# LuisaGroup/LuisaRender

Hardware: AMD Instinct MI355X
Metric: Msamples/s (+ fraction of HBM roofline) at fixed SPP, 1/2/4/8 GPU (higher is better)
Workload: dtype f32; 1 GPU; Contemporary Bathroom-class (procedural stand-in, ~600k tris), 1024x1024, 1024spp, depth 16; integrator=MegaPath, sampler=Independent (seed 19980810), spp=1024, parallelism=single GPU, collective=none (single GPU), scheduler=path pool, two contexts per lane (megapool_kernel.h)

## Files before the change

__graft_entry__.py:

```python
import os
import subprocess
import sys

ROOT = os.path.dirname(os.path.abspath(__file__))
if ROOT not in sys.path:
    sys.path.insert(0, ROOT)


def build() -> None:
    jobs = f"-j{min(os.cpu_count() or 4, 16)}"
    subprocess.check_call(["make", "-C", ROOT, jobs, "host", "oracle", "hip", "cli", "ieee", "shallow", "noearly", "nopair", "noride", "nostraight"])
    if os.path.isdir("/root/reference/src"):
        subprocess.check_call(["make", "-C", ROOT, jobs, "ref"])
    import luisarender_amd
    from luisarender_amd import _ffi
    _ffi.host_lib()
    assert os.path.exists(os.path.join(ROOT, "luisarender_amd", "lib", "liblrhip.so"))


def smoke() -> None:
    import numpy as np
    from luisarender_amd import Scene
    from oracle.check import Oracle
    from luisarender_amd.render import MegaPathRenderer
    from luisarender_amd.scenes import cornell_box

    scene = Scene.from_string(cornell_box(resolution=64, spp=8))
    renderer = MegaPathRenderer(0)
    renderer.upload(scene)
    renderer.render(0, 8, counters=True, sync=True)
    gpu = renderer.download(converted=False)
    cpu, counters = Oracle(scene).render(0, 8)
    rel = float(np.abs(gpu[..., :3] - cpu[..., :3]).sum() / np.abs(cpu[..., :3]).sum())
    gc = renderer.counters()
    assert np.array_equal(gpu[..., 3], cpu[..., 3]), "sample counts differ"
    assert abs(gc["closest_rays"] - counters["closest_rays"]) <= 2, (gc, counters)
    assert rel < 1e-4, f"relative L1 vs oracle {rel}"
    print(f"smoke ok: rel L1 vs oracle = {rel:.3e}, {renderer.last_render_ms():.3f} ms")


if __name__ == "__main__":
    build()
    if len(sys.argv) > 1 and sys.argv[1] == "smoke":
        smoke()
```

luisarender_amd/csrc/hip/lrhip_render.hip:

```cpp
#include "lrhip_internal.h"

namespace lrh {

#ifndef LR_TAPER_BIG
#define LR_TAPER_BIG 2.5
#endif
#ifndef LR_TAPER_SMALL
#define LR_TAPER_SMALL 3.0
#endif
#ifndef LR_TAPER_FRACTION
#define LR_TAPER_FRACTION 0.9
#endif
Chunking chunking_of(uint32_t spp, double shard_tiles, double item_scale, bool taper) {
    const auto s_opt = std::max(1.0, std::sqrt(item_scale * spp * shard_tiles / kNominalWaves));
    Chunking c{};
    if (taper && spp >= 16u) {
        const auto big_min = static_cast<long>((static_cast<uint64_t>(spp) * 2u + kMaxChunks - 1u) / kMaxChunks);
        c.big = static_cast<uint32_t>(std::clamp(std::max(std::lround(LR_TAPER_BIG * s_opt), big_min), 1l, static_cast<long>(spp)));
        c.small = static_cast<uint32_t>(std::clamp(std::lround(s_opt / LR_TAPER_SMALL), 1l, static_cast<long>(c.big)));
        c.big_count = static_cast<uint32_t>(std::floor(LR_TAPER_FRACTION * spp / c.big));
        const auto rest = spp - c.big_count * c.big;
        auto small_count = (rest + c.small - 1u) / c.small;
        if (c.big_count + small_count > kMaxChunks && c.big_count < kMaxChunks) {
            c.small = (rest + (kMaxChunks - c.big_count) - 1u) / (kMaxChunks - c.big_count);
            small_count = (rest + c.small - 1u) / c.small;
        }
        c.count = c.big_count + small_count;
        if (c.big_count >= 1u && small_count >= 1u && c.count <= kMaxChunks) { return c; }
    }
    auto count = static_cast<uint32_t>(std::lround(spp / s_opt));
    count = std::max(1u, std::min({count, spp, kMaxChunks}));
    c.count = c.big_count = count, c.big = (spp + count - 1u) / count, c.small = c.big;
    return c;
}

constexpr int kMinFixedBits = 24;
int fixed_point_bits(float film_clamp, float shutter_weight, uint32_t spp) {
    const auto bound = std::max(1.0, static_cast<double>(film_clamp) * std::max(1.0,
        std::fabs(static_cast<double>(shutter_weight)))) * std::max(1u, spp);
    if (!std::isfinite(bound)) { return -1; }
    const auto bits = std::min(40, 61 - static_cast<int>(std::ceil(std::log2(bound))));
    return bits >= kMinFixedBits ? bits : -1;
}
int ensure_accum(lrhip_ctx *ctx, uint32_t pixel_count) {
    const auto bytes = static_cast<size_t>(pixel_count) * 3u * sizeof(unsigned long long);
    if (ctx->wf_accum.bytes < bytes) {
        if (auto r = ensure(ctx->wf_accum, bytes); r != LRHIP_OK) { return r; }
        LR_HIP_CHECK(hipMemsetAsync(ctx->wf_accum.ptr, 0, bytes, ctx->stream));
    }
    return LRHIP_OK;
}
constexpr uint32_t kPoolAutoTriangles = 98304u;
uint32_t pool_auto_triangles(uint32_t max_depth, uint32_t scene_spp) {
    auto t = kPoolAutoTriangles;
    if (max_depth <= 6u) { t *= 2u; }
    if (scene_spp != 0u && scene_spp < 64u) { t /= 2u; }
    return t;
}
bool wants_pool(const lrhip_ctx *ctx) {
    return ctx->scheduler == 2u || (ctx->scheduler == 0u && ctx->update_counts[1] >= pool_auto_triangles(ctx->scene.max_depth,
        ctx->scene.sampler_spp));
}
int ensure_pool(lrhip_ctx *ctx, uint32_t resident_blocks) {
    return ensure(ctx->pool, static_cast<size_t>(resident_blocks) * lrd::kWavesPerBlock * lrd::kPoolSlots * lrd::kPoolRecordQuadsMax
        * sizeof(float4));
}

}

using namespace lrh;

extern "C" {

int lrhip_render(lrhip_ctx *ctx, const lrhip_render_params *p) {
    if (ctx == nullptr || p == nullptr || !ctx->scene_ready) { return fail(LRHIP_ERROR_INVALID, "lrhip_render: no scene uploaded"); }
    auto tiles_x = (ctx->width + 7u) / 8u, tiles_y = (ctx->height + 7u) / 8u;
    auto tile_count = tiles_x * tiles_y;
    if (p->spp_end < p->spp_begin || p->tile_stride == 0u || p->tile_end > tile_count) {
        return fail(LRHIP_ERROR_INVALID, "lrhip_render: invalid spp/tile range");
    }
    LR_HIP_CHECK(hipSetDevice(ctx->device));
    ctx->timed = false;
    if (p->spp_end == p->spp_begin || p->tile_begin >= p->tile_end) { return LRHIP_OK; }
    if (!ctx->scene.has_lights && ctx->scene.env_kind == lrd::kEnvNone && ctx->scene.integrator_kind != LR_INTEGRATOR_NORMAL) {
        return LRHIP_OK;
    }
    auto tiles_in_range = (p->tile_end - p->tile_begin + p->tile_stride - 1u) / p->tile_stride;
    auto spp = p->spp_end - p->spp_begin;
    const auto weight = (p->flags & LRHIP_RENDER_SHUTTER_WEIGHT) != 0u ? p->shutter_weight : 1.f;
    const auto fixed_bits = fixed_point_bits(ctx->scene.film_clamp, weight, spp);
    PlanInputs in{};
    in.features = ctx->features, in.force_features = ctx->diag_force_features, in.sampler_kind = ctx->scene.sampler_kind;
    in.wf_mode = ctx->wf_mode, in.max_depth = ctx->scene.max_depth;
    in.count = (p->flags & LRHIP_RENDER_COUNTERS) != 0u, in.env_tree = ctx->env_tree, in.byte_texels = ctx->packed_texel_words != 0u;
    in.wants_pool = wants_pool(ctx), in.fixed_fits = fixed_bits >= 0;
    if (fixed_bits < 0 && !ctx->in_split && fixed_point_bits(ctx->scene.film_clamp, weight, 1u) >= 0) {
        auto fitting = in;
        fitting.fixed_fits = true;
        if (plan_kernels(fitting).fixed_point) {
            auto n = spp;
            while (n > 1u && fixed_point_bits(ctx->scene.film_clamp, weight, n) < 0) { n = (n + 1u) / 2u; }
            LR_HIP_CHECK(hipEventRecord(ctx->ev_begin, ctx->stream));
            struct SplitGuard {
                lrhip_ctx *c;
                ~SplitGuard() { c->in_split = false; }
            } guard{ctx};
            ctx->in_split = true;
            auto rc = LRHIP_OK;
            for (auto s0 = p->spp_begin; s0 < p->spp_end && rc == LRHIP_OK; s0 += n) {
                auto sub = *p;
                sub.spp_begin = s0, sub.spp_end = std::min(p->spp_end, s0 + n);
                rc = lrhip_render(ctx, &sub);
            }
            return rc;
        }
    }
    const auto plan = plan_kernels(in);
    if (plan.family == LRHIP_FAMILY_WAVEFRONT) { return render_wavefront(ctx, p, plan, tiles_x, tiles_y, tiles_in_range, tile_count); }
    auto shard_tiles = static_cast<double>(tile_count) / std::max(p->balance_shards, 1u);
    auto item_scale = 1.25;
    if (ctx->diag_item_scale != 0.) { item_scale *= std::max(0.01, std::fabs(ctx->diag_item_scale)); }
    const auto ck = chunking_of(spp, shard_tiles, item_scale, ctx->diag_item_scale >= 0.);
    const auto chunk_count = ck.count;
    lrd::RenderArgs args{};
    args.film = ctx->film;
    ctx->scene.shutter_weight = weight;
    args.spp_begin = p->spp_begin, args.spp_end = p->spp_end;
    args.tile_begin = p->tile_begin, args.tile_end = p->tile_end, args.tile_stride = p->tile_stride;
    args.tiles_x = tiles_x, args.tiles_y = tiles_y;
    args.chunk_count = chunk_count;
    args.chunk_big_count = ck.big_count, args.chunk_big = ck.big, args.chunk_small = ck.small;
    args.item_count = tiles_in_range * chunk_count;
    args.work_counter = static_cast<uint32_t *>(ctx->work_counter.ptr);
    args.spill = static_cast<uint32_t *>(ctx->spill.ptr);
    args.counters = static_cast<lrd::DCounters *>(ctx->counters.ptr);
    auto pixel_count = ctx->width * ctx->height;
    LR_HIP_CHECK(hipMemsetAsync(ctx->work_counter.ptr, 0, 1024u, ctx->stream));
    const auto aov = plan.family == LRHIP_FAMILY_AOV, pool = plan.family == LRHIP_FAMILY_POOL;
    const auto entry = plan.family != LRHIP_FAMILY_NONE ? find_kernel(plan.main) : nullptr;
    if (entry == nullptr) {
        if (aov) {
            return fail(LRHIP_ERROR_UNSUPPORTED, "lrhip_render: no AOV kernel for feature mask " + std::to_string(plan.main)
                + " was compiled into this library");
        }
        return fail(LRHIP_ERROR_UNSUPPORTED, "lrhip_render: no megakernel variant for feature mask " + std::to_string(ctx->features) +
                                                 " was compiled into this library");
    }
    const auto aov_channels = aov ? ctx->scene.aov_channels : 0u;
// ... 58 lines not shown
```

luisarender_amd/csrc/hip/megapool_kernel.h:

```cpp
#pragma once
#include "dev_wavefront.h"

namespace lrd {

#ifndef LR_MIN_WAVES
#define LR_MIN_WAVES 4
#endif
#ifndef LR_POOL_SHADE_LANES
#define LR_POOL_SHADE_LANES 56
#endif
#ifndef LR_POOL_IDLE_LANES
#define LR_POOL_IDLE_LANES 16
#endif
#ifndef LR_POOL_TURNOVER_LANES
#define LR_POOL_TURNOVER_LANES 12
#endif
#ifndef LR_POOL_PARK_ON_STACK
#define LR_POOL_PARK_ON_STACK 1
#endif
#ifndef LR_POOL_FUSED_FETCH
#define LR_POOL_FUSED_FETCH 1
#endif
#ifndef LR_POOL_FUSED_ALPHA
#define LR_POOL_FUSED_ALPHA 0
#endif
#ifndef LR_POOL_EARLY_FETCH
#define LR_POOL_EARLY_FETCH 1
#endif
#ifndef LR_POOL_LEAF_NODE_PAIR
#define LR_POOL_LEAF_NODE_PAIR 1
#endif
#ifndef LR_POOL_EARLY_TAIL_PRIO
#define LR_POOL_EARLY_TAIL_PRIO 3
#endif
#ifndef LR_POOL_STATE_LEAN
#define LR_POOL_STATE_LEAN 1
#endif
#ifndef LR_POOL_RAY_INIT
#define LR_POOL_RAY_INIT if (!mine)
#endif
#ifndef LR_POOL_SHADOW_RIDE
#define LR_POOL_SHADOW_RIDE 1
#endif
constexpr uint32_t kPoolSlots = 128u;

template<bool GENERIC>
constexpr uint32_t pool_quads() { return GENERIC ? 5u : 4u; }
constexpr uint32_t kPoolRecordQuadsMax = pool_quads<true>() + 1u;
constexpr uint32_t kPoolPending = 1u << 22u;

enum : uint32_t {
    kCtxShadow = 1u, kCtxClosest = 2u,
    kCtxHadShadow = 4u, kCtxHadClosest = 8u,
    kCtxDone = 16u,
    kCtxOccluded = 32u,
    kCtxSide = 64u,
    kCtxOpen = 128u,
};
struct PathCtx {
    f3 so, sd;
    float s_tmax;
    f3 no, nd;
    float n_tmin, n_tmax;
    uint32_t tri;
    float u, v;
    uint32_t flags;
};
LR_D void ctx_start(PathCtx &c, TravState &tr) {
    tr.o = c.no, tr.d = c.nd, tr.t_min = c.n_tmin, tr.t_max = c.n_tmax;
    tr.phase = kPhaseClosest;
    if ((c.flags & kCtxShadow) != 0u) {
        asm volatile("");
        tr.o = c.so, tr.d = c.sd, tr.t_min = 0.f, tr.t_max = c.s_tmax;
        tr.phase = kPhaseShadow;
        c.flags &= ~kCtxShadow;
    } else {
        asm volatile("");
        c.flags &= ~kCtxClosest;
    }
    tr.cur = 0u, tr.sp = 0u;
    tr.hit.tri = kInvalid, tr.hit.u = 0.f, tr.hit.v = 0.f;
    tr.occluded = false;
}

LR_D void swap_words(float &x, float &y) { asm volatile("v_swap_b32 %0, %1" : "+v"(x), "+v"(y)); }
LR_D void swap_words(uint32_t &x, uint32_t &y) { asm volatile("v_swap_b32 %0, %1" : "+v"(x), "+v"(y)); }
LR_D void ctx_swap(PathCtx &a, PathCtx &b) {
    swap_words(a.so.x, b.so.x), swap_words(a.so.y, b.so.y), swap_words(a.so.z, b.so.z), swap_words(a.s_tmax, b.s_tmax);
    swap_words(a.sd.x, b.sd.x), swap_words(a.sd.y, b.sd.y), swap_words(a.sd.z, b.sd.z);
    swap_words(a.no.x, b.no.x), swap_words(a.no.y, b.no.y), swap_words(a.no.z, b.no.z), swap_words(a.n_tmin, b.n_tmin);
    swap_words(a.nd.x, b.nd.x), swap_words(a.nd.y, b.nd.y), swap_words(a.nd.z, b.nd.z), swap_words(a.n_tmax, b.n_tmax);
    swap_words(a.tri, b.tri), swap_words(a.u, b.u), swap_words(a.v, b.v), swap_words(a.flags, b.flags);
}

#ifndef LR_POOL_TURNOVER_MOVES
#define LR_POOL_TURNOVER_MOVES 1
#endif
LR_D void ctx_turnover(PathCtx &a, PathCtx &b) {
    if (LR_POOL_TURNOVER_MOVES == 0) { ctx_swap(a, b); return; }
    a.so = b.so, a.sd = b.sd, a.s_tmax = b.s_tmax, a.n_tmin = b.n_tmin, a.n_tmax = b.n_tmax;
    b.tri = a.tri, b.u = a.u, b.v = a.v;
    swap_words(a.no.x, b.no.x), swap_words(a.no.y, b.no.y), swap_words(a.no.z, b.no.z);
    swap_words(a.nd.x, b.nd.x), swap_words(a.nd.y, b.nd.y), swap_words(a.nd.z, b.nd.z);
    swap_words(a.flags, b.flags);
}

LR_D uint32_t lane_rank(unsigned long long mask) {
    return __builtin_amdgcn_mbcnt_hi(static_cast<uint32_t>(mask >> 32u), __builtin_amdgcn_mbcnt_lo(static_cast<uint32_t>(mask), 0u));
}

constexpr uint32_t kCtxRays = kCtxShadow | kCtxClosest;
LR_D bool ctx_shadeable(uint32_t flags, bool samples_left) {
#ifdef LR_POOL_SINGLE
    if ((flags & kCtxSide) != 0u) { samples_left = false; }
#endif
    return (flags & kCtxDone) != 0u || (samples_left && (flags & kCtxOpen) == 0u);
}
LR_D bool pool_shade_due(uint32_t phase, uint32_t cur_flags, uint32_t oth_flags, bool samples_left) {
    const auto idle = phase == kPhaseIdle;
    const auto s = lr_ballot(ctx_shadeable(oth_flags, samples_left) || (idle && ctx_shadeable(cur_flags, samples_left)));
    if (s == 0ull) { return false; }
    const auto idle_mask = lr_ballot(idle);
    return static_cast<uint32_t>(__popcll(s)) >= static_cast<uint32_t>(LR_POOL_SHADE_LANES) ||
           static_cast<uint32_t>(__popcll(s & idle_mask)) >= static_cast<uint32_t>(LR_POOL_IDLE_LANES) || idle_mask == ~0ull;
}

template<bool COUNT, bool ALPHA>
// ... 57 lines not shown
            stats.steps_starved += static_cast<uint32_t>(__builtin_readcyclecounter() - probe_t2);
        }
#endif
        if (n_ended == 0u) { continue; }
        if (n_ended < static_cast<uint32_t>(LR_POOL_TURNOVER_LANES) && lr_any(tr.cur < kCurParked)) { continue; }
        if (ended) {
            if (tr.phase == kPhaseShadow) {
                if (tr.occluded) { cur.flags |= kCtxOccluded; }
            } else {
                cur.tri = tr.hit.tri, cur.u = tr.hit.u, cur.v = tr.hit.v;
            }
            tr.phase = kPhaseIdle, tr.cur = kCurIdle;
            if ((cur.flags & kCtxRays) == 0u) {
                cur.flags |= kCtxDone;
                if ((oth.flags & kCtxRays) != 0u) { ctx_turnover(cur, oth); }
            }
            if ((cur.flags & kCtxRays) != 0u) {
                ctx_start(cur, tr);
                inv = safe_inverse(tr.d);
                spb = tl.lds_base;
            }
        }
        if (!lr_any(ended && tr.cur == kCurIdle)) { continue; }
        if (lr_ballot(tr.cur != kCurIdle) == 0ull) { break; }
        if (pool_shade_due(tr.phase, cur.flags, oth.flags, samples_left)) { break; }
    }
    if (EARLY != 0) { trav_fetch_wait(); }
    LR_MARK(kProbeTail, tr.cur);
    prio_shade();
    tr.sp = tl.sp_of(spb);
    return for_alpha;
}

#ifndef LR_PADDED_DRAWS_OUT_OF_LINE
#define LR_PADDED_DRAWS_OUT_OF_LINE 1
#endif
struct PaddedDraws {
    float a, b, c, d;
};
[[maybe_unused]] static __device__ __noinline__ PaddedDraws padded_draws(const DScene *scene, uint32_t sample_index, uint32_t pixel, uint32_t dimension, bool four) {
    PathSampler<true> sampler{};
    uint32_t words[kWfSamplerWordsMax] = {sample_index, 0u, dimension, pixel};
    sampler.restore(*scene, words);
    PaddedDraws r;
    r.a = sampler.next_1d();
    const auto u = sampler.next_2d();
    r.b = u.x, r.c = u.y;
    r.d = four ? sampler.next_1d() : 0.f;
    return r;
}

#ifndef LR_LIGHT_OUT_OF_LINE
#if defined(LR_VARIANT) && ((LR_VARIANT) & 16) && !((LR_VARIANT) & (96 | 256))
#define LR_LIGHT_OUT_OF_LINE 1
#else
#define LR_LIGHT_OUT_OF_LINE 0
#endif
#endif
template<bool ENV>
[[maybe_unused]] static __device__ __noinline__ LightPick sample_one_light_call(const DScene *scene, f3 p, f3 ng, f3 ns, uint32_t offset_bits, float u0, float u1, float u2) {
    SurfacePoint it{};
    it.p = p, it.ng = ng, it.shading.n = ns, it.offset_bits = offset_bits;
    return sample_one_light<ENV>(*scene, it, u0, f2{u1, u2});
}

#define LR_POOL_FILM_ADD(L, PIXEL, OF_ITEM, TILE_PIXEL)                                                                                          \
    do {                                                                                                                                         \
        const auto rgb = (L) * scene.shutter_weight;                                                                                             \
        if (CONT || (OF_ITEM) != item) {                                \
            wf_film_accumulate(scene, args.film, (PIXEL), rgb, scene.film_clamp);                                                                \
        } else if (!(any_nan(rgb) || any_inf(rgb))) {   \
            const auto threshold = scene.film_clamp * fmaxf(1.f, 1.f);                                                                           \
            const auto strength = fmaxf(fmaxf(fmaxf(fabsf(rgb.x), fabsf(rgb.y)), fabsf(rgb.z)), 0.f);                                            \
            const auto c = rgb * (threshold / fmaxf(strength, threshold));                                                                       \
            const auto px_sums = film_tile + (TILE_PIXEL) * 3u;                                                                                  \
            if (c.x != 0.f) { atomicAdd(px_sums + 0, radiance_to_fixed(c.x, scene.wf.accum_scale)); }                                            \
            if (c.y != 0.f) { atomicAdd(px_sums + 1, radiance_to_fixed(c.y, scene.wf.accum_scale)); }                                            \
            if (c.z != 0.f) { atomicAdd(px_sums + 2, radiance_to_fixed(c.z, scene.wf.accum_scale)); }                                            \
        } else {                                                                        \
            atomicAdd(&args.film[(PIXEL)].w, -1.f);                                                                                              \
        }                                                                                                                                        \
    } while (false)

template<uint32_t F>
__global__ __launch_bounds__(kBlockThreads, LR_MIN_WAVES) void megapool_kernel(DScenePtr scene_ptr, RenderArgs args) {
    const DScene &scene = *(const DScene *)scene_ptr;
    constexpr bool COUNT = (F & kFeatCount) != 0u, PCG = (F & kFeatGeneric) != 0u, ENV = (F & kFeatEnv) != 0u,
                   ALPHA = (F & kFeatAlpha) != 0u, DISNEY = (F & kFeatDisney) != 0u, WF = (F & kFeatWf) != 0u, CONT = (F & kFeatCont) != 0u;
    static_assert((F & kFeatPool) != 0u, "a pool variant");
    static_assert(kPoolParkedWords == 5u, "the shading block parks five words on top of a lane's stack (below): lrhip_upload_scene bounds the BVH depth with this constant");
    static_assert((F & (kFeatMix | kFeatLayered | kFeatAux | kFeatVpt | kFeatNest)) == 0u, "the pool scheduler exists for the lean kernels (closures inline)");
    static_assert(!WF || !DISNEY, "a wavefront variant is a lean kernel: the heavy closures live in heavy_kernel.h");
    static_assert(!CONT || WF, "the continuation pass exists in wavefront mode only");
    constexpr uint32_t SAMPLER_WORDS = PathSampler<PCG>::kSavedWords;
#ifdef LR_ONLY_SAMPLER
    constexpr bool PADDED = PCG && (LR_ONLY_SAMPLER) == LR_SAMPLER_PADDED_SOBOL;
#else
    constexpr bool PADDED = false;
#endif
    static_assert(PADDED == ((F & kFeatPadded) != 0u) || (F & kFeatPadded) == 0u, "a kFeatPadded kernel: generic sampler, LR_ONLY_SAMPLER = PaddedSobol");
    constexpr uint32_t QUADS = PADDED ? 4u : pool_quads<PCG>();
    constexpr bool RIDE = LR_POOL_SHADOW_RIDE != 0 && !WF;
    constexpr uint32_t RECORD = QUADS + (RIDE ? 1u : 0u);
    static_assert(RECORD <= kPoolRecordQuadsMax, "ensure_pool sizes the records");
    __shared__ uint32_t s_stack[kStackLds * kBlockThreads];
    __shared__ float4 s_stage[kWavesPerBlock * kStageWave];
#if LR_POOL_PARK_ON_STACK == 0
    __shared__ uint32_t s_park[5u * kBlockThreads];
    static_assert(kStackLds + 5u <= 16u, "the parking area is carved out of the round 1-3 stack: compile such pool variants with LR_STACK_LDS <= 11");
#endif
    __shared__ unsigned long long s_film[CONT ? 1u : kWavesPerBlock * 192u];
#ifdef LR_STALL_PROBE
    __shared__ uint32_t s_probe[kWavesPerBlock * kProbeWords];
    if ((threadIdx.x & 63u) < kProbeWords) { s_probe[(threadIdx.x >> 6u) * kProbeWords + (threadIdx.x & 63u)] = 0u; }
    const auto probe_wave = (F & kFeatCount) != 0u && (blockIdx.x % 9u) == 0u && __builtin_amdgcn_readfirstlane(threadIdx.x >> 6u) == ((blockIdx.x / 9u) & 3u);
#endif
    const auto tid = threadIdx.x;
    const auto lane = tid & 63u;
    const auto gtid = blockIdx.x * kBlockThreads + tid;
    const auto wave_in_block = __builtin_amdgcn_readfirstlane(tid >> 6u);
    TraversalStack stack{s_stack + tid, args.spill + gtid, args.total_threads, s_stage + wave_in_block * kStageWave};
    const auto film_tile = s_film + (CONT ? 0u : wave_in_block * 192u);
    const auto state_of = [&](uint32_t side, uint32_t quad) { return args.pool + static_cast<size_t>(side * RECORD + quad) * args.total_threads + gtid; };
    const auto state_load = [&](uint32_t side, uint32_t quad) { return *state_of(side, quad); };
    const auto state_store = [&](uint32_t side, uint32_t quad, float4 v) { *state_of(side, quad) = v; };
    DCounters local{};
    const auto t_wave = COUNT ? __builtin_readcyclecounter() : 0ull;

    const auto cont_total = CONT ? min(scene.wf.counts[kWfCountCont], scene.wf.capacity) : 0u;
    const auto cont_waves = gridDim.x * kWavesPerBlock;
    const auto item_records = CONT ? min(kWfItemRecords, max(64u, ((cont_total + cont_waves - 1u) / cont_waves + 63u) & ~63u)) : 1u;
    const auto item_count = CONT ? (cont_total + item_records - 1u) / item_records : args.item_count;
    const auto cont_queue = wf_cont_queue(scene);

    auto item = kInvalid;
    auto items_left = true;
    auto q_next = 0u, q_total = 0u;
    auto s_begin = 0u, s_count = 0u, tx = 0u, ty = 0u;
    if (!CONT) { film_tile[lane * 3u] = 0ull, film_tile[lane * 3u + 1u] = 0ull, film_tile[lane * 3u + 2u] = 0ull; }
    TravState tr{};
    tr.phase = kPhaseIdle;
    PathCtx cur{}, oth{};
    cur.flags = 0u, oth.flags = kCtxSide;

    auto flush_tile = [&]() {
        if (CONT || item == kInvalid) { return; }
        __builtin_amdgcn_fence(__ATOMIC_ACQ_REL, "wavefront");
        __builtin_amdgcn_wave_barrier();
        const auto a0 = film_tile[lane * 3u], a1 = film_tile[lane * 3u + 1u], a2 = film_tile[lane * 3u + 2u];
        film_tile[lane * 3u] = 0ull, film_tile[lane * 3u + 1u] = 0ull, film_tile[lane * 3u + 2u] = 0ull;
        const auto wx = tx * 8u + (lane & 7u), wy = ty * 8u + (lane >> 3u);
        if (wx < scene.camera.width && wy < scene.camera.height) {
            const auto index = wy * scene.camera.width + wx;
            const auto acc = scene.wf.accum + static_cast<size_t>(index) * 3u;
            if (a0 != 0ull) { atomicAdd(acc + 0, a0); }
            if (a1 != 0ull) { atomicAdd(acc + 1, a1); }
            if (a2 != 0ull) { atomicAdd(acc + 2, a2); }
            if (s_count != 0u) { atomicAdd(&args.film[index].w, static_cast<float>(s_count)); }
        }
        __builtin_amdgcn_fence(__ATOMIC_ACQ_REL, "wavefront");
        __builtin_amdgcn_wave_barrier();
    };

    auto take_item = [&]() {
        flush_tile();
        item = next_item(CONT ? scene.wf.counts + kWfWorkCont : args.work_counter, item_count, lane);
        q_next = 0u, q_total = 0u, s_count = 0u;
        if (item == kInvalid) {
            items_left = false;
            return;
        }
        if (CONT) {
            q_total = min(item_records, cont_total - item * item_records);
        } else {
            const auto range = item_range(args, item);
            const auto tile = args.tile_begin + range.tile_index * args.tile_stride;
            ty = tile / args.tiles_x, tx = (tile - ty * args.tiles_x + ty) % args.tiles_x;
            s_begin = range.s_begin, s_count = range.s_end > range.s_begin ? range.s_end - range.s_begin : 0u;
            q_total = s_count * 64u;
        }
    };

    for (;;) {
        for (;;) {
            const auto samples_left = items_left || q_next < q_total;
            if (!pool_shade_due(tr.phase, cur.flags, oth.flags, samples_left)) { break; }
            const auto t_shade = COUNT ? __builtin_readcyclecounter() : 0ull;
            if (ALPHA) { tr.pend_t = 0.f, tr.pend_u = 0.f, tr.pend_v = 0.f; }
            if (tr.phase == kPhaseIdle && !ctx_shadeable(oth.flags, samples_left)) { ctx_swap(cur, oth); }
#ifdef LR_POOL_SINGLE
            const auto mine = (oth.flags & kCtxDone) != 0u || ((oth.flags & kCtxOpen) == 0u && (oth.flags & kCtxSide) == 0u);
#else
            const auto mine = (oth.flags & kCtxDone) != 0u || (oth.flags & kCtxOpen) == 0u;
#endif
            {
                const auto stage = stack.stage;
                stage[lane] = make_float4(cur.so.x, cur.so.y, cur.so.z, cur.s_tmax);
                stage[64u + lane] = make_float4(cur.sd.x, cur.sd.y, cur.sd.z, cur.n_tmin);
                stage[128u + lane] = make_float4(cur.no.x, cur.no.y, cur.no.z, cur.n_tmax);
                const auto keep_word = (tr.phase & 7u) | (tr.occluded ? 8u : 0u) | (tr.sp << 5u) | (cur.flags << 12u) | (oth.flags << 20u);
                stage[192u + lane] = make_float4(cur.nd.x, cur.nd.y, cur.nd.z, __uint_as_float(keep_word));
#if LR_POOL_PARK_ON_STACK
                stack.push(tr.sp + 0u, tr.phase != kPhaseIdle ? tr.hit.tri : cur.tri);
                stack.push(tr.sp + 1u, __float_as_uint(tr.phase != kPhaseIdle ? tr.hit.u : cur.u));
                stack.push(tr.sp + 2u, __float_as_uint(tr.phase != kPhaseIdle ? tr.hit.v : cur.v));
                stack.push(tr.sp + 3u, __float_as_uint(tr.t_max));
                stack.push(tr.sp + 4u, tr.cur);
#else
                const auto park = s_park + tid;
                park[0u * kBlockThreads] = tr.phase != kPhaseIdle ? tr.hit.tri : cur.tri;
                park[1u * kBlockThreads] = __float_as_uint(tr.phase != kPhaseIdle ? tr.hit.u : cur.u);
                park[2u * kBlockThreads] = __float_as_uint(tr.phase != kPhaseIdle ? tr.hit.v : cur.v);
                park[3u * kBlockThreads] = __float_as_uint(tr.t_max);
                park[4u * kBlockThreads] = tr.cur;
#endif
                asm volatile("" ::: "memory");
            }
            PathSampler<PCG> sampler{};
            Ray ray{}, shadow{};
            LR_POOL_RAY_INIT {
                shadow.o = oth.so, shadow.d = oth.sd, shadow.t_min = 0.f, shadow.t_max = oth.s_tmax;
                ray.o = oth.no, ray.d = oth.nd, ray.t_min = oth.n_tmin, ray.t_max = oth.n_tmax;
            }
            f3 beta = mk3(0.f), Li = mk3(0.f), nee = mk3(0.f);
            auto pdf_bsdf = 1e16f;
            auto dp = 0u, pixel_index = 0u, path_item = kInvalid;
            const auto side = (oth.flags & kCtxSide) != 0u ? 1u : 0u;
            auto path_open = (oth.flags & kCtxDone) != 0u;
            const auto traced_shadow = path_open && (oth.flags & kCtxHadShadow) != 0u, traced_closest = path_open && (oth.flags & kCtxHadClosest) != 0u;
            const auto occluded = (oth.flags & kCtxOccluded) != 0u;
            const auto ro = oth.no, rd = oth.nd;
            const auto hit_tri = oth.tri;
            const auto hit_u = oth.u, hit_v = oth.v;
            constexpr bool LEAN_STATE = LR_POOL_STATE_LEAN != 0;
            auto word0 = 0u;
            const auto load_ids = [&]() {
                const auto q3 = state_load(side, 3u);
                pixel_index = __float_as_uint(q3.x), path_item = __float_as_uint(q3.y);
            };
            const auto sampler_take = [&](uint32_t stage) {
                if (PADDED) {
                    const auto q3 = state_load(side, 3u);
                    const auto depth = dp & 0xffffu;
                    const auto first_rr = scene.rr_depth == 0u ? 0u : scene.rr_depth - 1u;
                    const auto dimension = (scene.camera.kind == LR_CAMERA_THIN_LENS ? 4u : 2u) + 6u * depth + (depth > first_rr ? depth - first_rr : 0u) + 3u * stage;
                    uint32_t words[kWfSamplerWordsMax] = {__float_as_uint(q3.z), 0u, dimension, __float_as_uint(q3.w)};
                    sampler.restore(scene, words);
                    return;
                }
                const auto q3 = state_load(side, 3u);
                uint32_t words[kWfSamplerWordsMax] = {word0, __float_as_uint(q3.z), __float_as_uint(q3.w), __float_as_uint(state_load(side, QUADS - 1u).x)};
                sampler.restore(scene, words);
            };
            const auto sampler_leave = [&]() {
                if (PADDED) { return; }
                uint32_t words[kWfSamplerWordsMax] = {0u, 0u, 0u, 0u};
                sampler.save(words);
                word0 = words[0];
                state_store(side, 2u, make_float4(Li.x, Li.y, Li.z, __uint_as_float(words[0])));
                const auto q3 = state_load(side, 3u);
                state_store(side, 3u, make_float4(q3.x, q3.y, __uint_as_float(words[1]), __uint_as_float(words[2])));
                state_store(side, QUADS - 1u, make_float4(__uint_as_float(words[3]), 0.f, 0.f, 0.f));
            };
            auto sampler_left = false;
            if (path_open) {
                const auto q0 = state_load(side, 0u), q1 = state_load(side, 1u), q2 = state_load(side, 2u);
                nee = mk3(q0.x, q0.y, q0.z), pdf_bsdf = q0.w;
                beta = mk3(q1.x, q1.y, q1.z);
                const auto packed = __float_as_uint(q1.w);
                dp = packed & (RIDE ? 0x7fffffu : 0x3fffffu);
                Li = mk3(q2.x, q2.y, q2.z);
                word0 = __float_as_uint(q2.w);
                if (!LEAN_STATE) { load_ids(); }
                if (!PCG) {
                    uint32_t words[kWfSamplerWordsMax] = {word0, 0u, 0u, 0u};
                    sampler.restore(scene, words);
                }
            }
            auto want_shadow = false, want_closest = false;
            unsigned long long t_closure_sum = 0ull;
#ifdef LR_STALL_PROBE
            uint32_t t_lobe = 0u, t_eval = 0u, t_sample = 0u, t_hit = 0u, t_light = 0u;
            const auto probe_clock = []() { return static_cast<uint32_t>(__builtin_readcyclecounter()); };
            const auto t_block = probe_clock();
#endif
            auto park_kind = kInvalid;
            if (path_open) {
                if (traced_shadow) {
                    if (!occluded) { Li += nee; }
                }
                if (RIDE && (dp & kPoolPending) != 0u) {
                    const auto ids = state_load(side, QUADS);
                    LR_POOL_FILM_ADD(Li, __float_as_uint(ids.x), __float_as_uint(ids.y), __float_as_uint(ids.z));
                    Li = mk3(0.f), nee = mk3(0.f);
                    dp &= ~kPoolPending;
                }
                if (traced_closest) {
                    if (COUNT) { local.shade_busy++; }
                    const auto wo = -rd;
// ... 95 lines not shown
#endif
                        const LobeTables tables{scene.closures, scene.surfaces, scene.textures, scene.texels};
                        DClosure closure;
                        Frame sh;
                        load_lobe(tables, it.uv, it.ng, wo, (it.tags >> 12u) & 4095u, it.shading, closure, sh);
#ifdef LR_STALL_PROBE
                        asm volatile("" : "+v"(closure.c0[0]), "+v"(closure.s0), "+v"(sh.n.x));
                        const auto t_l1 = probe_clock();
                        t_lobe = t_l1 - static_cast<uint32_t>(t_closure);
#endif
                        if (pick.pdf > 0.0f) {
                            const auto eval = closure_evaluate<DISNEY>(closure, sh, it.ng, wo, shadow.d);
                            const auto w = balance(pick.pdf, eval.pdf) / pick.pdf;
                            nee = w * beta * eval.f * pick.L;
                            want_shadow = nee.x != 0.f || nee.y != 0.f || nee.z != 0.f;
                        }
#ifdef LR_STALL_PROBE
                        asm volatile("" : "+v"(nee.x), "+v"(nee.y), "+v"(nee.z));
                        const auto t_e1 = probe_clock();
                        t_eval = t_e1 - t_l1;
#endif
                        if constexpr (PADDED && LR_PADDED_DRAWS_OUT_OF_LINE != 0) {
                            sampler_take(1u);
                            const auto r = padded_draws(&scene, sampler.lo, sampler.w3, sampler.w2, rr);
                            u_lobe = r.a, u_bsdf = f2{r.b, r.c}, u_rr = r.d;
                        } else {
                            if (PCG) { sampler_take(1u); }
                            u_lobe = sampler.next_1d();
                            u_bsdf = sampler.next_2d();
                            if (PCG) {
                                if (rr) { u_rr = sampler.next_1d(); }
                                sampler_leave();
                            }
                        }
                        const auto bs = closure_sample<DISNEY>(closure, sh, it.ng, wo, u_lobe, u_bsdf);
                        auto eta = 1.f;
                        const auto has_eta = closure_eta(closure, eta);
                        ray.o = robust_origin(it, bs.wi);
                        ray.d = bs.wi;
                        ray.t_min = 0.f, ray.t_max = kFloatMax;
                        pdf_bsdf = bs.pdf;
                        beta *= (bs.pdf > 0.f ? 1.f / bs.pdf : 0.f) * bs.f;
                        auto eta_scale = 1.f;
                        if (has_eta) {
                            if (bs.event == kEventEnter) { eta_scale = sqr(eta); }
                            else if (bs.event == kEventExit) { eta_scale = sqr(1.f / eta); }
                        }
                        if (any_nan(beta)) { beta = mk3(0.f); }
                        auto alive = !(beta.x <= 0.f && beta.y <= 0.f && beta.z <= 0.f);
                        if (!PCG && rr) { u_rr = sampler.next_1d(); }
                        if (alive) {
                            const auto q = fmaxf(max_component(beta) * eta_scale, .05f);
                            if (rr) {
                                if (q < scene.rr_threshold && u_rr >= q) { alive = false; }
                                else { beta *= q < scene.rr_threshold ? 1.0f / q : 1.f; }
                            }
                        }
                        dp++;
                        want_closest = alive && (dp & 0xffffu) < scene.max_depth;
                        if (COUNT) { t_closure_sum += __builtin_readcyclecounter() - t_closure; }
#ifdef LR_STALL_PROBE
                        asm volatile("" : "+v"(beta.x), "+v"(ray.d.x));
                        t_sample = probe_clock() - t_e1;
#endif
                    }
                }
            }
            if (WF) {
                if (park_kind != kInvalid) { path_open = false; }
            }
            if (path_open && !want_shadow && !want_closest) {
                if (LEAN_STATE) { load_ids(); }
                LR_POOL_FILM_ADD(Li, pixel_index, path_item, dp >> 16u);
                path_open = false;
            }
            const auto t_regen = COUNT ? __builtin_readcyclecounter() : 0ull;
            if (COUNT) {
                for (auto off = 32; off > 0; off >>= 1) { t_closure_sum = max(t_closure_sum, static_cast<unsigned long long>(__shfl_xor(static_cast<long long>(t_closure_sum), off))); }
            }
            const auto final_shadow = RIDE && path_open && want_shadow && !want_closest;
            auto need = mine && (!path_open || final_shadow);
            auto got = false;
            auto new_k = 0u, new_item = kInvalid, new_px = 0u, new_py = 0u, new_s = 0u;
            for (;;) {
                const auto mask = lr_ballot(need);
                if (mask == 0ull) { break; }
                if (q_next >= q_total) {
                    if (!items_left) { break; }
                    take_item();
                    if (!items_left) { break; }
                    continue;
                }
                const auto avail = q_total - q_next;
                const auto rank = lane_rank(mask);
                if (need && rank < avail) {
                    const auto k = q_next + rank;
                    const auto px = tx * 8u + (k & 7u), py = ty * 8u + ((k >> 3u) & 7u);
                    if (CONT || (px < scene.camera.width && py < scene.camera.height)) {
                        new_k = k, new_item = item, new_px = px, new_py = py, new_s = s_begin + (k >> 6u);
                        got = true, need = false;
                    }
                }
                q_next += min(static_cast<uint32_t>(__popcll(mask)), avail);
            }
            if (got) {
                sampler_left = false;
                if (CONT) {
                    const auto rec = new_item * item_records + new_k;
                    const auto &q = cont_queue;
                    ray.o = q.get3(rec, 0u), ray.d = q.get3(rec, 3u);
                    ray.t_min = 0.f, ray.t_max = kFloatMax;
                    shadow.o = q.get3(rec, 6u), shadow.d = q.get3(rec, 9u);
                    shadow.t_min = 0.f, shadow.t_max = q.getf(rec, 12u);
                    nee = q.get3(rec, 13u), beta = q.get3(rec, 16u), Li = q.get3(rec, 19u);
                    pdf_bsdf = q.getf(rec, 22u);
                    pixel_index = q.get(rec, 23u);
                    const auto packed = q.get(rec, 24u);
                    dp = packed & 0xffffu;
                    want_shadow = (packed & (1u << 16u)) != 0u, want_closest = (packed & (1u << 17u)) != 0u;
                    uint32_t words[kWfSamplerWordsMax];
#pragma unroll
                    for (auto w = 0u; w < SAMPLER_WORDS; w++) { words[w] = q.get(rec, kWfContWords + w); }
                    sampler.restore(scene, words);
                    path_open = true;
                } else {
                    if (final_shadow) {
                        if (LEAN_STATE) { load_ids(); }
                        state_store(side, QUADS, make_float4(__uint_as_float(pixel_index), __uint_as_float(path_item), __uint_as_float(dp >> 16u), 0.f));
                    }
                    pixel_index = new_py * scene.camera.width + new_px;
                    path_item = new_item;
                    sampler.start(scene, new_px, new_py, new_s);
                    const auto u_filter = sampler.next_pixel_2d();
                    const auto u_lens = scene.camera.kind == LR_CAMERA_THIN_LENS ? sampler.next_2d() : f2{.5f, .5f};
                    float weight;
                    camera_ray(scene, scene.filter, new_px, new_py, u_filter, u_lens, ray, weight);
                    beta = mk3(weight);
                    if (!final_shadow) { Li = mk3(0.f), nee = mk3(0.f); }
                    pdf_bsdf = 1e16f;
                    dp = ((new_k & 63u) << 16u) | (final_shadow ? kPoolPending : 0u);
                    path_open = true, want_shadow = final_shadow, want_closest = true;
                    if (COUNT) { local.paths++; }
                }
            }
            const auto t_launch = COUNT ? __builtin_readcyclecounter() : 0ull;
            const auto go = path_open && (want_shadow || want_closest);
            if (go) {
                state_store(side, 0u, make_float4(nee.x, nee.y, nee.z, pdf_bsdf));
                state_store(side, 1u, make_float4(beta.x, beta.y, beta.z, __uint_as_float(dp)));
                if (!PCG || !sampler_left) {
                    uint32_t words[kWfSamplerWordsMax] = {word0, 0u, 0u, 0u};
                    if (!PCG || got) { sampler.save(words); }
                    state_store(side, 2u, make_float4(Li.x, Li.y, Li.z, __uint_as_float(words[0])));
                    if (got && PADDED) {
                        state_store(side, 3u, make_float4(__uint_as_float(pixel_index), __uint_as_float(path_item), __uint_as_float(words[0]), __uint_as_float(words[3])));
                    } else if (got) {
                        state_store(side, 3u, make_float4(__uint_as_float(pixel_index), __uint_as_float(path_item), __uint_as_float(words[1]), __uint_as_float(words[2])));
                        if (PCG) { state_store(side, QUADS - 1u, make_float4(__uint_as_float(words[3]), 0.f, 0.f, 0.f)); }
                    } else if (!LEAN_STATE && !PCG) {
                        state_store(side, 3u, make_float4(__uint_as_float(pixel_index), __uint_as_float(path_item), 0.f, 0.f));
                    }
                }
                if (COUNT) { local.closest_rays += want_closest ? 1u : 0u, local.shadow_rays += want_shadow ? 1u : 0u; }
            }
            {
                const auto stage = stack.stage;
                asm volatile("" ::: "memory");
                const auto p0 = stage[lane], p1 = stage[64u + lane], p2 = stage[128u + lane], p3 = stage[192u + lane];
                cur.so = mk3(p0.x, p0.y, p0.z), cur.s_tmax = p0.w;
                cur.sd = mk3(p1.x, p1.y, p1.z), cur.n_tmin = p1.w;
                cur.no = mk3(p2.x, p2.y, p2.z), cur.n_tmax = p2.w;
                cur.nd = mk3(p3.x, p3.y, p3.z);
                const auto keep_word = __float_as_uint(p3.w);
                tr.phase = keep_word & 7u, tr.occluded = (keep_word & 8u) != 0u;
                tr.sp = (keep_word >> 5u) & 127u;
#if LR_POOL_PARK_ON_STACK
                const auto keep_tri = stack.pop(tr.sp + 0u);
                const auto keep_u = __uint_as_float(stack.pop(tr.sp + 1u)), keep_v = __uint_as_float(stack.pop(tr.sp + 2u));
                tr.t_max = __uint_as_float(stack.pop(tr.sp + 3u)), tr.cur = stack.pop(tr.sp + 4u);
#else
                const auto park = s_park + tid;
                const auto keep_tri = park[0u * kBlockThreads];
                const auto keep_u = __uint_as_float(park[1u * kBlockThreads]), keep_v = __uint_as_float(park[2u * kBlockThreads]);
                tr.t_max = __uint_as_float(park[3u * kBlockThreads]), tr.cur = park[4u * kBlockThreads];
#endif
                cur.flags = (keep_word >> 12u) & 0xffu, cur.tri = keep_tri, cur.u = keep_u, cur.v = keep_v;
                tr.hit.tri = keep_tri, tr.hit.u = keep_u, tr.hit.v = keep_v;
                __builtin_amdgcn_fence(__ATOMIC_ACQ_REL, "wavefront");
                oth.so = shadow.o, oth.sd = shadow.d, oth.s_tmax = shadow.t_max;
                oth.no = ray.o, oth.nd = ray.d, oth.n_tmin = ray.t_min, oth.n_tmax = ray.t_max;
                oth.tri = kInvalid, oth.u = 0.f, oth.v = 0.f;
                const auto shaded_flags = (side != 0u ? kCtxSide : 0u) |
                                          (go ? kCtxOpen | (want_shadow ? kCtxShadow | kCtxHadShadow : 0u) | (want_closest ? kCtxClosest | kCtxHadClosest : 0u) : 0u);
                oth.flags = mine ? shaded_flags : (keep_word >> 20u) & 0xffu;
                if ((tr.phase & 3u) == kPhaseShadow) { tr.o = cur.so, tr.d = cur.sd, tr.t_min = 0.f; }
                else { tr.o = cur.no, tr.d = cur.nd, tr.t_min = cur.n_tmin; }
            }
            if (tr.phase == kPhaseIdle && (oth.flags & kCtxRays) != 0u) {
                ctx_swap(cur, oth);
                ctx_start(cur, tr);
            }
#ifdef LR_STALL_PROBE
            if (COUNT) {
                const auto wave_max = [](uint32_t v) {
                    for (auto off = 32; off > 0; off >>= 1) { v = max(v, static_cast<uint32_t>(__shfl_xor(static_cast<int>(v), off))); }
                    return v;
                };
                const auto m_hit = wave_max(t_hit), m_light = wave_max(t_light), m_lobe = wave_max(t_lobe), m_eval = wave_max(t_eval), m_sample = wave_max(t_sample);
                if (probe_wave && lane == 0u) {
                    atomicAdd(&args.counters->probe[14], 1ull);
                    atomicAdd(&args.counters->probe[15], static_cast<unsigned long long>(probe_clock() - t_block));
                    atomicAdd(&args.counters->probe[8], static_cast<unsigned long long>(m_hit + m_light));
                    atomicAdd(&args.counters->probe[9], static_cast<unsigned long long>(m_lobe));
                    atomicAdd(&args.counters->probe[10], static_cast<unsigned long long>(m_eval));
                    atomicAdd(&args.counters->probe[11], static_cast<unsigned long long>(m_sample));
                }
            }
#endif
            if (COUNT) {
                if (lane == 0u) {
                    const auto t_end = __builtin_readcyclecounter();
                    local.shade_cycles += t_end - t_shade;
                    local.shade_closure_cycles += t_closure_sum, local.shade_regen_cycles += t_launch - t_regen;
                    local.shade_light_cycles += (t_regen - t_shade) - t_closure_sum;
                }
                local.shade_calls++;
            }
        }
        if (!lr_any(tr.phase != kPhaseIdle)) { break; }
        TraceStats ts{};
#ifdef LR_STALL_PROBE
        ts.probe_lds = probe_wave ? static_cast<uint32_t>(reinterpret_cast<uintptr_t>((TraversalStack::lds_u32 *)(s_probe + wave_in_block * kProbeWords))) : 0u;
#endif
        const auto t_trace = COUNT ? __builtin_readcyclecounter() : 0ull;
        for (;;) {
            const auto for_alpha = pool_trace<COUNT, ALPHA>(scene, stack, tr, cur, oth, items_left || q_next < q_total, ts);
            if (!ALPHA) { break; }
            if (lr_any((tr.phase & kPhasePendingAlpha) != 0u)) { resolve_pending_alpha(scene, stack, tr); }
            if (!for_alpha) { break; }
        }
#ifdef LR_STALL_PROBE
        if (COUNT && ts.probe_lds != 0u && lane == 0u) {
            const auto words = s_probe + wave_in_block * kProbeWords;
#pragma unroll
            for (auto i = 0u; i < kProbeSlots; i++) { atomicAdd(&args.counters->probe[i], static_cast<unsigned long long>(words[i])), words[i] = 0u; }
            atomicAdd(&args.counters->probe[12], static_cast<unsigned long long>(ts.steps));
            atomicAdd(&args.counters->probe[13], static_cast<unsigned long long>(__builtin_readcyclecounter() - t_trace));
        }
#endif
        if (COUNT) {
            if (lane == 0u) { local.trace_cycles += __builtin_readcyclecounter() - t_trace; }
            local.nodes_visited += ts.nodes, local.tris_tested += ts.tris, local.nodes_empty += ts.nodes_empty;
            local.trace_steps += ts.steps, local.trace_steps_busy += ts.steps_busy, local.trace_steps_starved += ts.steps_starved;
#ifndef LR_STALL_PROBE
            if (ts.early_fetch_broken != 0u) { atomicAdd(&args.counters->probe[kProbeEarlyFetchBroken], static_cast<unsigned long long>(ts.early_fetch_broken)); }
#endif
        }
    }
    flush_tile();

    if (COUNT) {
        if (lane == 0u) { local.wave_cycles = __builtin_readcyclecounter() - t_wave; }
        auto reduce = [&](unsigned long long v, unsigned long long *dst) {
            for (auto off = 32; off > 0; off >>= 1) { v += __shfl_down(v, off); }
            if (lane == 0u) { atomicAdd(dst, v); }
        };
        reduce(local.paths, &args.counters->paths);
        reduce(local.closest_rays, &args.counters->closest_rays);
        reduce(local.shadow_rays, &args.counters->shadow_rays);
        reduce(local.nodes_visited, &args.counters->nodes_visited);
        reduce(local.tris_tested, &args.counters->tris_tested);
        reduce(local.surface_hits, &args.counters->surface_hits);
        reduce(local.nee_samples, &args.counters->nee_samples);
        reduce(local.path_length_sum, &args.counters->path_length_sum);
        reduce(local.trace_steps, &args.counters->trace_steps);
        reduce(local.trace_steps_busy, &args.counters->trace_steps_busy);
        reduce(local.shade_calls, &args.counters->shade_calls);
        reduce(local.shade_busy, &args.counters->shade_busy);
        reduce(local.trace_steps_starved, &args.counters->trace_steps_starved);
        reduce(local.shade_cycles, &args.counters->shade_cycles);
        reduce(local.trace_cycles, &args.counters->trace_cycles);
        reduce(local.wave_cycles, &args.counters->wave_cycles);
        reduce(local.nodes_empty, &args.counters->nodes_empty);
        reduce(local.shade_light_cycles, &args.counters->shade_light_cycles);
        reduce(local.shade_closure_cycles, &args.counters->shade_closure_cycles);
        reduce(local.shade_regen_cycles, &args.counters->shade_regen_cycles);
    }
}

#undef LR_POOL_FILM_ADD

}
```

Before: 1307 Msamples/s.

## Stash pre-generated camera rays per wave to decouple path regeneration

Adds a per-wave ring buffer in global memory that holds pre-generated camera ray records: origin, direction, weight, pixel, item and sampler state. The buffer is filled in a batched pass early in shading, and terminated lanes then pop from it instead of running the hand-out loop and camera sampling inline. The aim is to cut the divergent regeneration cost inside the shade step by generating rays for many lanes at once. In exchange it costs extra global-memory traffic and pool allocation, more register pressure, and extra complexity in tracking termination through samples_left.

```diff
diff --git a/__graft_entry__.py b/__graft_entry__.py
--- a/__graft_entry__.py
+++ b/__graft_entry__.py
@@ -9,7 +9,7 @@
 
 def build() -> None:
     jobs = f"-j{min(os.cpu_count() or 4, 16)}"
-    subprocess.check_call(["make", "-C", ROOT, jobs, "host", "oracle", "hip", "cli", "ieee", "shallow", "noearly", "nopair", "noride", "nostraight"])
+    subprocess.check_call(["make", "-C", ROOT, jobs, "host", "oracle", "hip", "cli", "ieee", "shallow", "noearly", "nopair", "noride", "nostash", "nostraight"])
     if os.path.isdir("/root/reference/src"):
         subprocess.check_call(["make", "-C", ROOT, jobs, "ref"])
     import luisarender_amd
diff --git a/luisarender_amd/csrc/hip/lrhip_render.hip b/luisarender_amd/csrc/hip/lrhip_render.hip
--- a/luisarender_amd/csrc/hip/lrhip_render.hip
+++ b/luisarender_amd/csrc/hip/lrhip_render.hip
@@ -62,8 +62,8 @@
         ctx->scene.sampler_spp));
 }
 int ensure_pool(lrhip_ctx *ctx, uint32_t resident_blocks) {
-    return ensure(ctx->pool, static_cast<size_t>(resident_blocks) * lrd::kWavesPerBlock * lrd::kPoolSlots * lrd::kPoolRecordQuadsMax
-        * sizeof(float4));
+    return ensure(ctx->pool, static_cast<size_t>(resident_blocks) * lrd::kWavesPerBlock
+        * (lrd::kPoolSlots * lrd::kPoolRecordQuadsMax + lrd::kPoolStashEntries * lrd::kPoolStashQuads) * sizeof(float4));
 }
 
 }
diff --git a/luisarender_amd/csrc/hip/megapool_kernel.h b/luisarender_amd/csrc/hip/megapool_kernel.h
--- a/luisarender_amd/csrc/hip/megapool_kernel.h
+++ b/luisarender_amd/csrc/hip/megapool_kernel.h
@@ -42,7 +42,12 @@
 #ifndef LR_POOL_SHADOW_RIDE
 #define LR_POOL_SHADOW_RIDE 1
 #endif
+#ifndef LR_POOL_PATH_STASH
+#define LR_POOL_PATH_STASH 1
+#endif
 constexpr uint32_t kPoolSlots = 128u;
+constexpr uint32_t kPoolStashEntries = 128u;
+constexpr uint32_t kPoolStashQuads = 4u;
 
 template<bool GENERIC>
 constexpr uint32_t pool_quads() { return GENERIC ? 5u : 4u; }
@@ -266,6 +271,29 @@
         }                                                                                                                                        \
     } while (false)
 
+#define LR_POOL_HAND_OUT()                                                                                                                       \
+            for (;;) {                                                                                                                           \
+                const auto mask = lr_ballot(need);                                                                                               \
+                if (mask == 0ull) { break; }                                                                                                     \
+                if (q_next >= q_total) {      \
+                    if (!items_left) { break; }                                                                                                  \
+                    take_item();                                                                                                                 \
+                    if (!items_left) { break; }                                                                                                  \
+                    continue;                                                                                                                    \
+                }                                                                                                                                \
+                const auto avail = q_total - q_next;                                                                                             \
+                const auto rank = lane_rank(mask);                                                                                               \
+                if (need && rank < avail) {                                                                                                      \
+                    const auto k = q_next + rank;                                                                                                \
+                    const auto px = tx * 8u + (k & 7u), py = ty * 8u + ((k >> 3u) & 7u);                                                         \
+                    if (CONT || (px < scene.camera.width && py < scene.camera.height)) {                                                         \
+                        new_k = k, new_item = item, new_px = px, new_py = py, new_s = s_begin + (k >> 6u);                                       \
+                        got = true, need = false;                                                                                                \
+                    }                                                                                                                            \
+                }                                                                                                                                \
+                q_next += min(static_cast<uint32_t>(__popcll(mask)), avail);                                                                     \
+            }
+
 template<uint32_t F>
 __global__ __launch_bounds__(kBlockThreads, LR_MIN_WAVES) void megapool_kernel(DScenePtr scene_ptr, RenderArgs args) {
     const DScene &scene = *(const DScene *)scene_ptr;
@@ -287,6 +315,8 @@
     constexpr bool RIDE = LR_POOL_SHADOW_RIDE != 0 && !WF;
     constexpr uint32_t RECORD = QUADS + (RIDE ? 1u : 0u);
     static_assert(RECORD <= kPoolRecordQuadsMax, "ensure_pool sizes the records");
+    constexpr bool STASH = LR_POOL_PATH_STASH != 0 && !WF && !ALPHA && !(ENV && PCG && !DISNEY) && !(ENV && DISNEY && !PCG && (F & kFeatByteTex) == 0u);
+    constexpr bool STASH_SCALAR_ITEM = STASH && !ENV;
     __shared__ uint32_t s_stack[kStackLds * kBlockThreads];
     __shared__ float4 s_stage[kWavesPerBlock * kStageWave];
 #if LR_POOL_PARK_ON_STACK == 0
@@ -322,6 +352,9 @@
     auto q_next = 0u, q_total = 0u;
     auto s_begin = 0u, s_count = 0u, tx = 0u, ty = 0u;
     if (!CONT) { film_tile[lane * 3u] = 0ull, film_tile[lane * 3u + 1u] = 0ull, film_tile[lane * 3u + 2u] = 0ull; }
+    [[maybe_unused]] auto stash_head = 0u, stash_count = 0u;
+    [[maybe_unused]] const auto stash = args.pool + static_cast<size_t>(2u * kPoolRecordQuadsMax) * args.total_threads +
+                                        static_cast<size_t>(blockIdx.x * kWavesPerBlock + wave_in_block) * (kPoolStashQuads * kPoolStashEntries);
     TravState tr{};
     tr.phase = kPhaseIdle;
     PathCtx cur{}, oth{};
@@ -349,6 +382,7 @@
     auto take_item = [&]() {
         flush_tile();
         item = next_item(CONT ? scene.wf.counts + kWfWorkCont : args.work_counter, item_count, lane);
+        if constexpr (STASH_SCALAR_ITEM) { item = static_cast<uint32_t>(__builtin_amdgcn_readfirstlane(static_cast<int>(item))); }
         q_next = 0u, q_total = 0u, s_count = 0u;
         if (item == kInvalid) {
             items_left = false;
@@ -367,7 +401,7 @@
 
     for (;;) {
         for (;;) {
-            const auto samples_left = items_left || q_next < q_total;
+            const auto samples_left = items_left || q_next < q_total || (STASH && stash_count != 0u);
             if (!pool_shade_due(tr.phase, cur.flags, oth.flags, samples_left)) { break; }
             const auto t_shade = COUNT ? __builtin_readcyclecounter() : 0ull;
             if (ALPHA) { tr.pend_t = 0.f, tr.pend_u = 0.f, tr.pend_v = 0.f; }
@@ -399,6 +433,36 @@
                 park[4u * kBlockThreads] = tr.cur;
 #endif
                 asm volatile("" ::: "memory");
+            }
+            [[maybe_unused]] uint32_t t_fill = 0u;
+            if constexpr (STASH) {
+                if (__builtin_amdgcn_readfirstlane(stash_count < static_cast<uint32_t>(__popcll(lr_ballot(mine))) && (items_left || q_next < q_total) ? 1 : 0) != 0) {
+                    const auto t_fill0 = COUNT ? __builtin_readcyclecounter() : 0ull;
+                    auto need = true, got = false;
+                    auto new_k = 0u, new_item = kInvalid, new_px = 0u, new_py = 0u, new_s = 0u;
+                    LR_POOL_HAND_OUT();
+                    const auto filled = lr_ballot(got);
+                    if (got) {
+                        const auto entry = stash + ((stash_head + stash_count + lane_rank(filled)) & (kPoolStashEntries - 1u));
+                        PathSampler<PCG> first{};
+                        first.start(scene, new_px, new_py, new_s);
+                        const auto u_filter = first.next_pixel_2d();
+                        const auto u_lens = scene.camera.kind == LR_CAMERA_THIN_LENS ? first.next_2d() : f2{.5f, .5f};
+                        Ray camera{};
+                        float weight;
+                        camera_ray(scene, scene.filter, new_px, new_py, u_filter, u_lens, camera, weight);
+                        uint32_t words[kWfSamplerWordsMax] = {0u, 0u, 0u, 0u};
+                        first.save(words);
+                        entry[0u * kPoolStashEntries] = make_float4(camera.o.x, camera.o.y, camera.o.z, camera.t_min);
+                        entry[1u * kPoolStashEntries] = make_float4(camera.d.x, camera.d.y, camera.d.z, camera.t_max);
+                        entry[2u * kPoolStashEntries] = make_float4(weight, __uint_as_float(new_py * scene.camera.width + new_px), __uint_as_float(new_item), __uint_as_float(new_k & 63u));
+                        entry[3u * kPoolStashEntries] = PADDED ? make_float4(__uint_as_float(words[0]), __uint_as_float(words[3]), 0.f, 0.f)
+                                                               : make_float4(__uint_as_float(words[0]), __uint_as_float(words[1]), __uint_as_float(words[2]), __uint_as_float(words[3]));
+                    }
+                    stash_count += static_cast<uint32_t>(__popcll(filled));
+                    __builtin_amdgcn_fence(__ATOMIC_ACQ_REL, "wavefront");
+                    if (COUNT) { t_fill = static_cast<uint32_t>(__builtin_readcyclecounter() - t_fill0); }
+                }
             }
             PathSampler<PCG> sampler{};
             Ray ray{}, shadow{};
@@ -660,27 +724,39 @@
             auto need = mine && (!path_open || final_shadow);
             auto got = false;
             auto new_k = 0u, new_item = kInvalid, new_px = 0u, new_py = 0u, new_s = 0u;
-            for (;;) {
+            if constexpr (STASH) {
                 const auto mask = lr_ballot(need);
-                if (mask == 0ull) { break; }
-                if (q_next >= q_total) {
-                    if (!items_left) { break; }
-                    take_item();
-                    if (!items_left) { break; }
-                    continue;
-                }
-                const auto avail = q_total - q_next;
-                const auto rank = lane_rank(mask);
-                if (need && rank < avail) {
-                    const auto k = q_next + rank;
-                    const auto px = tx * 8u + (k & 7u), py = ty * 8u + ((k >> 3u) & 7u);
-                    if (CONT || (px < scene.camera.width && py < scene.camera.height)) {
-                        new_k = k, new_item = item, new_px = px, new_py = py, new_s = s_begin + (k >> 6u);
+                if (mask != 0ull && stash_count != 0u) {
+                    const auto rank = lane_rank(mask);
+                    if (need && rank < stash_count) {
+                        const auto entry = stash + ((stash_head + rank) & (kPoolStashEntries - 1u));
+                        const auto e0 = entry[0u * kPoolStashEntries], e1 = entry[1u * kPoolStashEntries], e2 = entry[2u * kPoolStashEntries], e3 = entry[3u * kPoolStashEntries];
                         got = true, need = false;
+                        sampler_left = false;
+                        if (final_shadow) {
+                            if (LEAN_STATE) { load_ids(); }
+                            state_store(side, QUADS, make_float4(__uint_as_float(pixel_index), __uint_as_float(path_item), __uint_as_float(dp >> 16u), 0.f));
+                        }
+                        pixel_index = __float_as_uint(e2.y);
+                        path_item = __float_as_uint(e2.z);
+                        uint32_t words[kWfSamplerWordsMax] = {__float_as_uint(e3.x), 0u, 0u, 0u};
+                        if (PADDED) { words[3] = __float_as_uint(e3.y); }
+                        else if (PCG) { words[1] = __float_as_uint(e3.y), words[2] = __float_as_uint(e3.z), words[3] = __float_as_uint(e3.w); }
+                        sampler.restore(scene, words);
+                        ray.o = mk3(e0.x, e0.y, e0.z), ray.t_min = e0.w;
+                        ray.d = mk3(e1.x, e1.y, e1.z), ray.t_max = e1.w;
+                        beta = mk3(e2.x);
+                        if (!final_shadow) { Li = mk3(0.f), nee = mk3(0.f); }
+                        pdf_bsdf = 1e16f;
+                        dp = (__float_as_uint(e2.w) << 16u) | (final_shadow ? kPoolPending : 0u);
+                        path_open = true, want_shadow = final_shadow, want_closest = true;
+                        if (COUNT) { local.paths++; }
                     }
-                }
-                q_next += min(static_cast<uint32_t>(__popcll(mask)), avail);
-            }
+                    const auto taken = min(static_cast<uint32_t>(__popcll(mask)), stash_count);
+                    stash_head = (stash_head + taken) & (kPoolStashEntries - 1u), stash_count -= taken;
+                }
+            } else {
+            LR_POOL_HAND_OUT();
             if (got) {
                 sampler_left = false;
                 if (CONT) {
@@ -721,6 +797,7 @@
                     if (COUNT) { local.paths++; }
                 }
             }
+            }
             const auto t_launch = COUNT ? __builtin_readcyclecounter() : 0ull;
             const auto go = path_open && (want_shadow || want_closest);
             if (go) {
@@ -801,6 +878,7 @@
                     local.shade_cycles += t_end - t_shade;
                     local.shade_closure_cycles += t_closure_sum, local.shade_regen_cycles += t_launch - t_regen;
                     local.shade_light_cycles += (t_regen - t_shade) - t_closure_sum;
+                    if constexpr (STASH) { local.shade_regen_cycles += t_fill, local.shade_light_cycles -= t_fill; }
                 }
                 local.shade_calls++;
             }
@@ -812,7 +890,7 @@
 #endif
         const auto t_trace = COUNT ? __builtin_readcyclecounter() : 0ull;
         for (;;) {
-            const auto for_alpha = pool_trace<COUNT, ALPHA>(scene, stack, tr, cur, oth, items_left || q_next < q_total, ts);
+            const auto for_alpha = pool_trace<COUNT, ALPHA>(scene, stack, tr, cur, oth, items_left || q_next < q_total || (STASH && stash_count != 0u), ts);
             if (!ALPHA) { break; }
             if (lr_any((tr.phase & kPhasePendingAlpha) != 0u)) { resolve_pending_alpha(scene, stack, tr); }
             if (!for_alpha) { break; }
```

Result: faster. 1332 Msamples/s (median of 6 runs) (+1.9%).
